# supernomad/quantum

Hardware: AMD Instinct MI355X
Metric: AES-256-GCM seal+unseal GiB/s (device-resident packets) at 1/2/4/8 MI355X (higher is better)
Workload: dtype u8

## Files before the change

quantum_amd/csrc/gcm_kernels.hip:

```cpp
#include <hip/hip_runtime.h>
#include <stdint.h>

#include <algorithm>

#include "gcm_internal.h"

namespace qgcm {

typedef __attribute__((address_space(3))) uint32_t lds_u32;
typedef uint32_t u32x4 __attribute__((ext_vector_type(4)));
typedef __attribute__((address_space(3))) u32x4 lds_u128;

struct __attribute__((aligned(4))) W4 {
    uint32_t x, y, z, w;
};

#ifndef QGCM_NT_DATA
#define QGCM_NT_DATA 0
#endif
typedef uint32_t u32x4u __attribute__((ext_vector_type(4), aligned(4)));
__device__ __forceinline__ W4 load_block(const W4 *p) {
    if constexpr ((QGCM_NT_DATA & 1) != 0) {
        const u32x4u v = __builtin_nontemporal_load(reinterpret_cast<const u32x4u *>(p));
        return W4{v.x, v.y, v.z, v.w};
// ... 257 lines not shown
        }
        *(lds_u64 *)(size_t)(512u * i + 8u * v) = u32x2{a0, a1};
        *(lds_u64 *)(size_t)(512u * i + 256u + 8u * v) = u32x2{a2, a3};
    }
}

struct Tab2F {
    Keys kk;
    TT<kG5Bytes, true> t;
    uint32_t mf8;
    __device__ __forceinline__ void setup(Ctr &c, uint32_t n0, uint32_t n1, uint32_t n2, uint32_t hi) const {
        ctr_setup(c, n0, n1, n2, hi, kk, t);
    }
    __device__ __forceinline__ void block(const Ctr &c, uint32_t lo, uint32_t &k0, uint32_t &k1, uint32_t &k2,
                                          uint32_t &k3) const {
        ctr_block_t<TT<kG5Bytes, true>, kG5Bytes>(c, lo, kk, t, k0, k1, k2, k3);
    }
    __device__ __forceinline__ void ghash(uint32_t &y0, uint32_t &y1, uint32_t &y2, uint32_t &y3, uint32_t) const {
        ghash_mul5(y0, y1, y2, y3, mf8);
    }
};

__device__ __forceinline__ uint32_t vreg(uint32_t x) {
    asm volatile("" : "+v"(x));
    return x;
}

template <bool kFence = true>
__device__ __forceinline__ void ghash_mul(uint32_t &y0, uint32_t &y1, uint32_t &y2, uint32_t &y3, uint32_t gb) {
    uint32_t a0 = 0, a1 = 0, a2 = 0, a3 = 0;
    const uint32_t yw[4] = {y0, y1, y2, y3};
#pragma unroll
    for (int w = 0; w < 4; ++w) {
        const uint32_t hi = yw[w] & 0xf0f0f0f0u;
        const uint32_t lo = (yw[w] << 4) & 0xf0f0f0f0u;
#pragma unroll
        for (int k = 0; k < 4; ++k) {
            const int j = 4 * w + k;
            const uint4 th = lds128(perm(gb, hi, 0x0c060500u | k) + (2 * j) * 256);
            const uint4 tl = lds128(perm(gb, lo, 0x0c060500u | k) + (2 * j + 1) * 256);
            a0 = xor3(a0, th.x, tl.x);
            a1 = xor3(a1, th.y, tl.y);
            a2 = xor3(a2, th.z, tl.z);
            a3 = xor3(a3, th.w, tl.w);
        }
        if constexpr (kFence) asm volatile("" : "+v"(a0), "+v"(a1), "+v"(a2), "+v"(a3)::"memory");
    }
    y0 = a0;
    y1 = a1;
    y2 = a2;
    y3 = a3;
}

__device__ __forceinline__ void ghash_mul_global(uint32_t &y0, uint32_t &y1, uint32_t &y2, uint32_t &y3,
                                                 const uint4 *__restrict__ T) {
    uint32_t a0 = 0, a1 = 0, a2 = 0, a3 = 0;
    const uint32_t yw[4] = {y0, y1, y2, y3};
    const char *base = reinterpret_cast<const char *>(T);
#pragma unroll
    for (int w = 0; w < 4; ++w) {
#pragma unroll
        for (int k = 0; k < 4; ++k) {
            const int j = 4 * w + k;
            const uint32_t oh = (yw[w] >> (8 * k)) & 0xf0u;
            const uint32_t ol = ((yw[w] >> (8 * k)) & 0x0fu) << 4;
            const uint4 th = *reinterpret_cast<const uint4 *>(base + (2 * j) * 256 + oh);
            const uint4 tl = *reinterpret_cast<const uint4 *>(base + (2 * j + 1) * 256 + ol);
            a0 = xor3(a0, th.x, tl.x);
            a1 = xor3(a1, th.y, tl.y);
            a2 = xor3(a2, th.z, tl.z);
            a3 = xor3(a3, th.w, tl.w);
        }
        asm volatile("" : "+v"(a0), "+v"(a1), "+v"(a2), "+v"(a3)::"memory");
    }
    y0 = a0;
    y1 = a1;
    y2 = a2;
    y3 = a3;
}

__device__ __forceinline__ void ghash_lenblock_global(uint32_t aad_len, uint32_t L, const uint4 *__restrict__ T,
                                                      uint32_t &y0, uint32_t &y1, uint32_t &y2, uint32_t &y3) {
    const char *base = reinterpret_cast<const char *>(T);
    const uint32_t w1 = bswap(aad_len * 8u), w3 = bswap(L * 8u);
    const uint32_t v[5] = {w1 >> 24, w3, w3 >> 8, w3 >> 16, w3 >> 24};
    const int j[5] = {7, 12, 13, 14, 15};
    uint32_t a0 = 0, a1 = 0, a2 = 0, a3 = 0;
#pragma unroll
    for (int i = 0; i < 5; ++i) {
        const uint4 th = *reinterpret_cast<const uint4 *>(base + (2 * j[i]) * 256 + (v[i] & 0xf0u));
        const uint4 tl = *reinterpret_cast<const uint4 *>(base + (2 * j[i] + 1) * 256 + ((v[i] & 0x0fu) << 4));
        a0 = xor3(a0, th.x, tl.x);
        a1 = xor3(a1, th.y, tl.y);
        a2 = xor3(a2, th.z, tl.z);
        a3 = xor3(a3, th.w, tl.w);
    }
    y0 = a0;
    y1 = a1;
    y2 = a2;
    y3 = a3;
}

__device__ __forceinline__ uint32_t sel4(uint32_t q, uint32_t a, uint32_t b, uint32_t c, uint32_t d) {
    return q == 0 ? a : (q == 1 ? b : (q == 2 ? c : d));
}
__device__ __forceinline__ uint32_t lowmask(uint32_t s) { return s ? (0xffffffffu >> (32 - 8 * s)) : 0u; }
__device__ __forceinline__ void store_bytes(uint8_t *p, uint32_t v, uint32_t nbytes) {
    if (nbytes > 0) p[0] = (uint8_t)v;
    if (nbytes > 1) p[1] = (uint8_t)(v >> 8);
    if (nbytes > 2) p[2] = (uint8_t)(v >> 16);
}
__device__ __forceinline__ uint32_t load_bytes(const uint8_t *p, uint32_t nbytes) {
    uint32_t v = 0;
    if (nbytes > 0) v |= p[0];
    if (nbytes > 1) v |= (uint32_t)p[1] << 8;
    if (nbytes > 2) v |= (uint32_t)p[2] << 16;
    return v;
}


__device__ __forceinline__ void read_tail(const uint8_t *data, uint32_t L, uint32_t &g0, uint32_t &g1, uint32_t &g2,
                                          uint32_t &g3, uint32_t &n0, uint32_t &n1, uint32_t &n2) {
    const uint32_t s = L & 3u;
    const uint32_t *t = reinterpret_cast<const uint32_t *>(data + (L & ~3u));
    const uint32_t w0 = t[0], w1 = t[1], w2 = t[2], w3 = t[3], w4 = t[4], w5 = t[5], w6 = t[6];
    const uint32_t w7 = load_bytes(data + (L & ~3u) + 28, s);
    g0 = __builtin_amdgcn_alignbyte(w1, w0, s);
    g1 = __builtin_amdgcn_alignbyte(w2, w1, s);
    g2 = __builtin_amdgcn_alignbyte(w3, w2, s);
    g3 = __builtin_amdgcn_alignbyte(w4, w3, s);
    n0 = __builtin_amdgcn_alignbyte(w5, w4, s);
    n1 = __builtin_amdgcn_alignbyte(w6, w5, s);
    n2 = __builtin_amdgcn_alignbyte(w7, w6, s);
}

__device__ __forceinline__ void read_nonce(const uint8_t *data, uint32_t L, uint32_t &n0, uint32_t &n1, uint32_t &n2) {
    const uint32_t s = L & 3u;
    const uint32_t *t = reinterpret_cast<const uint32_t *>(data + (L & ~3u));
    const uint32_t w4 = t[4], w5 = t[5], w6 = t[6];
    const uint32_t w7 = load_bytes(data + (L & ~3u) + 28, s);
    n0 = __builtin_amdgcn_alignbyte(w5, w4, s);
    n1 = __builtin_amdgcn_alignbyte(w6, w5, s);
    n2 = __builtin_amdgcn_alignbyte(w7, w6, s);
}
// ... 77 lines not shown
        const W4 &c = kSeal ? out : in;
        eng.ghash(z0, z1, z2, z3, gH4);
        z0 ^= c.x;
        z1 ^= c.y;
        z2 ^= c.z;
        z3 ^= c.w;
        blast = (int)bi;
    }
    const bool part = r && (nfull & 3u) == m;
    if (part || m == (d & 3u)) {
        const uint32_t ctr = part ? nfull + 2 : 1u;
        if ((ctr >> 8) != hi) {
            hi = ctr >> 8;
            eng.setup(cc, n0, n1, n2, hi);
        }
        uint32_t k0, k1, k2, k3;
        eng.block(cc, ctr & 0xffu, k0, k1, k2, k3);
        if (part) {
            uint8_t *blk = data + 16u * nfull;
            const W4 in = *reinterpret_cast<const W4 *>(blk);
            const uint32_t q = r >> 2, sb = r & 3u;
            const uint32_t o0 = in.x ^ k0, o1 = in.y ^ k1, o2 = in.z ^ k2, o3 = in.w ^ k3;
            uint32_t *bw = reinterpret_cast<uint32_t *>(blk);
            if (q > 0) bw[0] = o0;
            if (q > 1) bw[1] = o1;
            if (q > 2) bw[2] = o2;
            const uint32_t oq = sel4(q, o0, o1, o2, o3) & lowmask(sb);
            W4 c = kSeal ? W4{o0, o1, o2, o3} : in;
            if (kSeal)
                prefix = oq;
            else
                store_bytes(blk + 4 * q, oq, sb);
            c.x &= q > 0 ? 0xffffffffu : lowmask(sb);
            c.y &= q > 1 ? 0xffffffffu : (q == 1 ? lowmask(sb) : 0u);
            c.z &= q > 2 ? 0xffffffffu : (q == 2 ? lowmask(sb) : 0u);
            c.w &= q == 3 ? lowmask(sb) : 0u;
            eng.ghash(z0, z1, z2, z3, gH4);
            z0 ^= c.x;
            z1 ^= c.y;
            z2 ^= c.z;
            z3 ^= c.w;
            blast = (int)nfull;
        } else {
            e0 = k0;
            e1 = k1;
            e2 = k2;
            e3 = k3;
        }
    }
    }
    {
        const uint32_t em = d + 1u - (uint32_t)blast;
        const uint32_t tsel = em == 2 ? kGhH2 : em == 3 ? kGhH3 : em == 4 ? kGhH4 : kGhH5;
        ghash_mul_global(z0, z1, z2, z3, Hg + tsel);
        uint32_t l0, l1, l2, l3;
        ghash_lenblock_global(b.aad_len, L, Hg, l0, l1, l2, l3);
        z0 = quad_xor(z0) ^ l0;
        z1 = quad_xor(z1) ^ l1;
        z2 = quad_xor(z2) ^ l2;
        z3 = quad_xor(z3) ^ l3;
    }
    e0 = quad_xor(e0);
    e1 = quad_xor(e1);
    e2 = quad_xor(e2);
    e3 = quad_xor(e3);
    const uint32_t t0 = z0 ^ e0, t1 = z1 ^ e1, t2 = z2 ^ e2, t3 = z3 ^ e3;
    const uint32_t owner = r ? (nfull & 3u) : 0u;
    if (kSeal) {
        if (m == owner) {
            write_tail(data, L, t0, t1, t2, t3, n0, n1, n2, prefix);
            if (b.status) b.status[pkt] = 1;
        }
    } else {
        read_tag(data, L, g0, g1, g2, g3);
        const bool ok = ((t0 ^ g0) | (t1 ^ g1) | (t2 ^ g2) | (t3 ^ g3)) == 0;
        if (!ok) {
            for (uint32_t bi = m; bi < nfull; bi += 4) {
                const W4 zz = {0, 0, 0, 0};
                *reinterpret_cast<W4 *>(data + 16u * bi) = zz;
            }
            if (r && m == owner) {
                uint32_t *bw = reinterpret_cast<uint32_t *>(data + 16u * nfull);
                for (uint32_t w = 0; w < (r >> 2); ++w) bw[w] = 0;
                store_bytes(data + 16u * nfull + (r & ~3u), 0, r & 3u);
            }
        }
        if (b.status && m == 0) b.status[pkt] = ok ? 1 : 0;
    }
}

#ifndef QGCM_TILE_POOL
#define QGCM_TILE_POOL 4
#endif
#ifndef QGCM_TAIL_EIGHTHS
#define QGCM_TAIL_EIGHTHS 4
#endif
constexpr uint32_t kPoolCtr = kG5Bytes + kTeBytes;

#ifdef QGCM_QUAD_STATS
__device__ unsigned long long g_quad_stats[4096 * 8];
#endif

template <bool kDesc>
constexpr int quad_waves() { return kDesc ? 12 : 16; }
template <bool kDesc>
constexpr int quad_wpe() { return kDesc ? 3 : 8; }

template <bool kSeal, bool kDesc>
__global__ void __launch_bounds__(quad_waves<kDesc>() * 64) __attribute__((amdgpu_waves_per_eu(quad_wpe<kDesc>(),
                                                                                                  quad_wpe<kDesc>())))
gcm_quad_kernel(Batch b, const uint32_t *__restrict__ rk_table) {
    constexpr uint32_t kW = quad_waves<kDesc>();
    constexpr uint32_t kT = kW * 64;
    constexpr uint32_t kTeBase = kDesc ? 0u : kG5Bytes;
    const uint32_t lane = threadIdx.x & 63u;
    const uint32_t wave = threadIdx.x >> 6;
    const uint32_t m = lane & 3u;
    const uint32_t qd = lane >> 2;
    if (kDesc && b.tile_list && __builtin_amdgcn_readfirstlane(*b.n_list) == 0) return;

    for (uint32_t i = threadIdx.x; i < kTeBytes / 4; i += kT) {
        const uint32_t x = i >> 6, slot = i & 63u;
        lds_st32(kTeBase + 4 * i, b.te[(slot >> 5) * 256u + x]);
    }
    if constexpr (!kDesc) g5_fill(b.gh_table + (size_t)b.uniform_key * kGhEntries + kGhH4, threadIdx.x, kT);
    if constexpr (!kDesc && QGCM_TILE_POOL) {
        if (threadIdx.x == 0) lds_st32(kPoolCtr, kW);
    }
#if QGCM_TILE_POOL == 4
    if constexpr (!kDesc) {
        if (threadIdx.x == 0) lds_st32(kPoolCtr + 12, 0u);
    }
#endif
    __syncthreads();

    const uint32_t lb = (lane & 31u) << 2;
    const uint32_t m8 = vreg(0x0000ff00u), mf8 = vreg(0x000000f8u);
    const uint32_t gH4 = kDesc ? kTeBytes + wave * kGhBytes : 0u;
    uint32_t cur_key = kDesc ? 0xffffffffu : b.uniform_key;
    const uint32_t ntiles = kDesc ? (b.tile_list ? *b.n_list : b.n_items >> 4) : ((b.n + 15) >> 4);

#ifdef QGCM_QUAD_STATS
    unsigned long long *qs = g_quad_stats + (size_t)blockIdx.x * 8u;
    uint32_t qs_tiles = 0;
    if (!kDesc && threadIdx.x == 0) {
        qs[0] = wall_clock64();
        qs[4] = __builtin_amdgcn_s_getreg((31 << 11) | 20);
        qs[5] = __builtin_amdgcn_s_getreg((31 << 11) | 4);
    }
#endif
#ifdef QGCM_QUAD_STATS
#define QS_TILE() ++qs_tiles
#define QS_END()                                                  \
    do {                                                          \
        if (!kDesc && lane == 0) {                                \
            const unsigned long long t_ = wall_clock64();         \
            atomicMax(&qs[1], t_);                                \
            atomicAdd(&qs[2], t_);                                \
            atomicAdd(&qs[3], (unsigned long long)qs_tiles);      \
            atomicMax(&qs[6], (1ull << 62) - t_);                 \
        }                                                         \
    } while (0)
#else
#define QS_TILE() do { } while (0)
#define QS_END() do { } while (0)
#endif
#if QGCM_TILE_POOL == 4
    uint32_t sidx = 0xffffffffu, tail0 = 0;
    if constexpr (!kDesc) {
        const uint32_t rows = ntiles / (gridDim.x * kW);
        if (b.pool && rows > 0) {
            const uint32_t tail_rows = rows < 2 ? 0u : std::min(rows - 1u, std::max(1u, rows * QGCM_TAIL_EIGHTHS / 8u));
            sidx = (rows - tail_rows) * kW;
            tail0 = (rows - tail_rows) * gridDim.x * kW;
        }
    }
#endif
    uint32_t tile = blockIdx.x * kW + wave;
    if constexpr (kDesc) {
        uint32_t t = 0;
        if (lane == 0) t = atomicAdd(b.tile_counter, 1u);
        tile = __builtin_amdgcn_readfirstlane(__shfl(t, 0));
    }
    for (; tile < ntiles;) {
        uint32_t pkt, L;
        bool valid;
        uint64_t off;
        uint32_t wkey = cur_key;
        if constexpr (kDesc) {
            const uint32_t wt = b.tile_list ? b.tile_list[tile] : tile;
            pkt = b.worklist[wt * 16u + qd];
            valid = pkt != 0xffffffffu;
            qgcm_desc dsc = {0, 0, 0};
            if (valid) dsc = b.descs[pkt];
            off = dsc.offset;
            L = kSeal ? dsc.len : dsc.len - QGCM_OVERHEAD;
            const uint64_t vmask = __ballot(valid);
            if (vmask != 0) {
                wkey = __builtin_amdgcn_readfirstlane(__shfl(dsc.key_idx, __ffsll((unsigned long long)vmask) - 1));
                if (wkey != cur_key) {
                    const uint4 *src = b.gh_table + (size_t)wkey * kGhEntries + kGhH4;
#pragma unroll
                    for (int r = 0; r < 8; ++r) {
                        const uint32_t e = r * 64 + lane;
                        lds_st_comb(gH4, e, src[e]);
                    }
                    __builtin_amdgcn_fence(__ATOMIC_RELEASE, "wavefront");
                    __builtin_amdgcn_wave_barrier();
                    __builtin_amdgcn_fence(__ATOMIC_ACQUIRE, "wavefront");
                    cur_key = wkey;
                }
            }
            uint32_t t = 0;
            if (lane == 0) t = atomicAdd(b.tile_counter, 1u);
            const uint32_t next = __builtin_amdgcn_readfirstlane(__shfl(t, 0));
            asm volatile("" : "+v"(L));
            if (!valid) {
                tile = next;
                continue;
            }
            tile = next;
        } else {
            pkt = tile * 16u + qd;
            L = b.uniform_len;
            asm volatile("" : "+s"(L));
            valid = pkt < b.n;
            if (!kSeal) {
                if (L < (uint32_t)QGCM_OVERHEAD) valid = false;
                L -= QGCM_OVERHEAD;
            }
            off = (uint64_t)pkt * b.stride;
            if constexpr (QGCM_TILE_POOL) {
                uint32_t i = 0;
                if (lane == 0) i = __atomic_fetch_add((lds_u32 *)(size_t)kPoolCtr, 1u, __ATOMIC_RELAXED);
                i = __builtin_amdgcn_readfirstlane(i);
                tile = blockIdx.x * kW + (i % kW) + (i / kW) * gridDim.x * kW;
#if QGCM_TILE_POOL == 4
                if (i >= sidx) {
                    uint32_t c = 0;
                    if (lane == 0) c = atomicAdd(b.pool, 1u);
                    tile = tail0 + __builtin_amdgcn_readfirstlane(c);
                }
#endif
            } else {
                tile += gridDim.x * kW;
            }
            if (!valid) {
                if (!kSeal && b.status && pkt < b.n && m == 0) b.status[pkt] = 0;
                continue;
            }
        }
        const Keys kk = {rk_table + (size_t)wkey * kRkWords, rk_table + (size_t)wkey * kRkWords + 64};
        if constexpr (kDesc) {
            quad_packet<kSeal>(b, Tab2{kk, {lb, m8}}, pkt, off, L, wkey, m, gH4);
        } else {
            quad_packet<kSeal>(b, Tab2F{kk, {lb, m8}, mf8}, pkt, off, L, wkey, m, gH4);
        }
        QS_TILE();
    }
    QS_END();
#if QGCM_TILE_POOL == 4
    if constexpr (!kDesc) {
        if (b.pool) {
            uint32_t last = 0;
            if (lane == 0 && __atomic_fetch_add((lds_u32 *)(size_t)(kPoolCtr + 12), 1u, __ATOMIC_RELAXED) == kW - 1) {
                __threadfence();
                last = atomicAdd(b.pool + kPoolDoneWord, 1u) == gridDim.x - 1u ? 1u : 0u;
            }
            if (lane == 0 && last) {
                __threadfence();
                b.pool[0] = 0;
                b.pool[kPoolDoneWord] = 0;
                __threadfence_system();
                __hip_atomic_store(b.pool_done, b.pool_gen, __ATOMIC_RELEASE, __HIP_MEMORY_SCOPE_SYSTEM);
            }
        }
    }
#endif
}
#undef QS_TILE
#undef QS_END

#ifdef QGCM_QUAD_STATS
extern "C" int qgcm_debug_quad_stats(unsigned long long *out, int n, int reset) {
    if (n > 4096 * 8) n = 4096 * 8;
    if (hipMemcpyFromSymbol(out, HIP_SYMBOL(g_quad_stats), (size_t)n * 8) != hipSuccess) return -1;
    if (reset) {
        static unsigned long long zero[4096 * 8];
        if (hipMemcpyToSymbol(HIP_SYMBOL(g_quad_stats), zero, sizeof(zero)) != hipSuccess) return -1;
    }
    return 0;
}
#endif

constexpr uint32_t kSegCtl = kG5Bytes + kTeBytes;
constexpr uint32_t kSegLds = kSegCtl + 16u;
constexpr uint32_t kSegDone = 0xffffffffu;

__device__ __forceinline__ volatile lds_u32 *seg_ctl(uint32_t i) { return (volatile lds_u32 *)(size_t)(kSegCtl + 4u * i); }

template <class P>
__device__ __forceinline__ uint32_t wave_lower_bound(uint32_t lo, uint32_t hi, uint32_t lane, P pred) {
    while (hi - lo > 63u) {
        const uint32_t step = (hi - lo + 62u) / 63u;
        const uint32_t p = min(lo + lane * step, hi);
        const uint64_t msk = __ballot(pred(p));
        const uint32_t f = (uint32_t)__ffsll((unsigned long long)msk) - 1u;
        if (f == 0) return lo;
        const uint32_t nlo = lo + (f - 1u) * step + 1u, nhi = min(lo + f * step, hi);
        lo = nlo;
        hi = nhi;
    }
    const uint64_t msk = __ballot(pred(min(lo + lane, hi)));
    return lo + (uint32_t)__ffsll((unsigned long long)msk) - 1u;
}

#ifdef QGCM_SEG_STATS
__device__ unsigned long long g_seg_stats[4096 * 16];
#define SEG_STAT_ADD(i, v) \
    do { if (lane == 0) atomicAdd(&g_seg_stats[blockIdx.x * 16u + (i)], (unsigned long long)(v)); } while (0)
#define SEG_NOW() wall_clock64()
#else
#define SEG_STAT_ADD(i, v) do { } while (0)
#define SEG_NOW() 0ull
#endif

#ifndef QGCM_SEG_START
#define QGCM_SEG_START 1
#endif
#ifndef QGCM_SEG_HELP_MIN
#define QGCM_SEG_HELP_MIN 16
#endif
#ifndef QGCM_SEG_LAST
// ... 1270 lines not shown
```

quantum_amd/csrc/qgcm_api.cpp:

```cpp
#include <hip/hip_runtime.h>
#include <errno.h>
#include <stdint.h>
#include <stdio.h>
#include <stdlib.h>
#include <string.h>
#include <sys/random.h>

#include <algorithm>
#include <atomic>
#include <chrono>
#include <memory>
#include <future>
#include <map>
#include <mutex>
#include <thread>
#include <vector>

#include "../../include/qgcm.h"
#include "chain_claim.h"
#include "gcm_internal.h"

using namespace qgcm;

constexpr int kPipeStreams = 3;
constexpr uint64_t kPipeChunk = 32ull << 20;
constexpr uint64_t kHostChunk = 64ull << 20;
constexpr uint64_t kHostRing = 4ull << 30;

struct qgcm_ctx {
    int device = 0;
    int num_cus = 0;
    uint32_t max_keys = 0;
    int uniform_variant = kVariantUniform;
    int desc_variant = kVariantDescQuad;
    int wgs_per_cu_override = 0;
    bool one_kernel = true;
    bool variant_forced = false;
    uint32_t desc_one_max = kDescOneMax;
    uint32_t direct_max = kDirectMax;
    uint32_t one_uniform_max = kOneUniformMax;
    uint32_t launch_chunk = kLaunchChunk;
    uint32_t desc_chunk = kDescChunk;
    bool desc_one_on = true, host_direct = true, small_wl = true;
    uint64_t chain_chunk = kPipeChunk;
    int chain_slots = kPipeStreams, chain_dev_ahead = 2, chain_dev_backlog = -1;
    bool snappy_group = true;
    int snappy_per_cu = 0;
    bool chain_pin = true;
    std::mutex codec_cpus_mu;
    std::vector<int> codec_cpus;
    uint32_t *d_rk = nullptr;
    uint4 *d_gh = nullptr;
    uint4 *d_pw = nullptr;
    uint32_t pw_keys = 0;
    uint32_t *d_te = nullptr;
    uint8_t *d_sbox = nullptr;
    uint8_t *d_key_valid = nullptr;
    std::vector<uint8_t> key_set;
    std::mutex key_mu;

    std::mutex ws_mu;
    void *d_qws = nullptr;
    size_t qws_cap = 0;

    std::mutex io_mu;
    struct OneSlot {
        std::mutex mu;
        hipStream_t stream = nullptr;
        uint8_t *h = nullptr;
        size_t cap = 0;
    };
    static constexpr int kOneSlots = 8;
    static constexpr size_t kOneSlotCap = kOneCap + 4096;
    static_assert((kOneCap - 16u) + 16u <= kOneSlotCap, "record, tail and status bytes fit a pooled staging slot");
    static_assert(one_fits_launch(16336, true, QGCM_MAX_AAD) && !one_fits_launch(16337, true, QGCM_MAX_AAD) &&
                      one_record_bytes(16336, true) + one_tail_bytes(QGCM_MAX_AAD) + 16u <= kOneSlotCap,
                  "the largest long-AAD call fits a pooled staging slot");
    OneSlot one[kOneSlots];
    OneSlot big;
    std::atomic<uint32_t> one_rr{0};

    hipStream_t pipe[kPipeStreams] = {};
    std::vector<hipEvent_t> ev_in, ev_kern, ev_out;
    uint64_t host_chunk = kHostChunk, host_ring = kHostRing;
    uint8_t *d_ring = nullptr;
    size_t ring_cap = 0;
    uint8_t *h_stat = nullptr;
    size_t hstat_cap = 0;
// ... 32 lines not shown

int env_int(const char *name, int dflt) {
    const char *v = getenv(name);
    return v && *v ? atoi(v) : dflt;
}

uint8_t gf8_mul(uint8_t a, uint8_t b) {
    uint8_t p = 0;
    for (int i = 0; i < 8; ++i) {
        if (b & 1) p ^= a;
        const uint8_t hi = a & 0x80;
        a <<= 1;
        if (hi) a ^= 0x1b;
        b >>= 1;
    }
    return p;
}

void build_tables(uint8_t sbox[256], uint32_t te[512]) {
    for (int x = 0; x < 256; ++x) {
        uint8_t inv = 0;
        if (x) {
            uint8_t r = 1, b = (uint8_t)x;
            for (int e = 254; e; e >>= 1) {
                if (e & 1) r = gf8_mul(r, b);
                b = gf8_mul(b, b);
            }
            inv = r;
        }
        auto rl = [](uint8_t v, int s) { return (uint8_t)((v << s) | (v >> (8 - s))); };
        sbox[x] = inv ^ rl(inv, 1) ^ rl(inv, 2) ^ rl(inv, 3) ^ rl(inv, 4) ^ 0x63;
    }
    for (int x = 0; x < 256; ++x) {
        const uint32_t s = sbox[x], s2 = gf8_mul((uint8_t)s, 2), s3 = s2 ^ s;
        const uint32_t t0 = s2 | (s << 8) | (s << 16) | (s3 << 24);
        te[x] = t0;
        te[256 + x] = (t0 << 8) | (t0 >> 24);
    }
}

void set_err(char *err, int errlen, const char *msg) {
    if (err && errlen > 0) snprintf(err, (size_t)errlen, "%s", msg);
}

int hip_fail(hipError_t e) { return e == hipSuccess ? QGCM_OK : QGCM_E_HIP; }

int grid_for(const qgcm_ctx *ctx, uint32_t n_items, int variant) {
    const int cus = std::max(1, ctx->num_cus - resident_workers_running(ctx->res.load(std::memory_order_acquire)));
    const uint32_t waves = (uint32_t)variant_waves(variant);
    const uint32_t tiles = (n_items + 15) / 16;
    const uint32_t wgs = (tiles + waves - 1) / waves;
    const uint32_t per_cu = ctx->wgs_per_cu_override > 0 ? (uint32_t)ctx->wgs_per_cu_override
                                                         : (uint32_t)variant_wgs_per_cu(variant);
    const uint32_t cap = (uint32_t)cus * per_cu;
    return (int)(wgs < cap ? (wgs ? wgs : 1) : cap);
}

Batch base_batch(const qgcm_ctx *ctx) {
    Batch b{};
    b.rk_table = ctx->d_rk;
    b.gh_table = ctx->d_gh;
    b.pw_table = ctx->d_pw;
    b.pw_keys = ctx->pw_keys;
    b.te = ctx->d_te;
    b.key_valid = ctx->d_key_valid;
    b.max_keys = ctx->max_keys;
    return b;
}

int run_uniform(qgcm_ctx *ctx, bool seal, uint8_t *arena, uint64_t stride, uint32_t n, uint32_t len,
                uint32_t key_idx, const uint8_t *nonces, uint32_t aad_len, uint8_t *status, hipStream_t s);

int run_one(qgcm_ctx *ctx, bool seal, uint8_t *slot, uint64_t stride, uint32_t len, uint32_t key_idx,
            uint32_t aad_len, uint8_t *status, hipStream_t s) {
    if (ctx->one_kernel && stride + one_tail_bytes(aad_len) <= kOneCap - 16 && !(stride & 15) &&
        !((uintptr_t)slot & 15)) {
        volatile uint8_t *done = status + 1;
        *done = 0;
        Batch b = base_batch(ctx);
        b.done = status + 1;
        b.arena = slot;
        b.status = status;
        b.stride = stride;
        b.uniform_len = len;
        b.uniform_key = key_idx;
        b.n = 1;
        b.n_items = 64;
        b.aad_len = aad_len;
        if (launch_one(seal, b, s) != hipSuccess) return QGCM_E_HIP;
        ctx->count(QGCM_KERNEL_ONE);
        const auto t0 = std::chrono::steady_clock::now();
        for (uint32_t spins = 0; *done == 0; ++spins) {
            __builtin_ia32_pause();
            if ((spins & 1023) == 1023 && std::chrono::steady_clock::now() - t0 > std::chrono::seconds(1)) break;
        }
        if (*done == 0) return hip_fail(hipStreamSynchronize(s));
        std::atomic_thread_fence(std::memory_order_acquire);
        return QGCM_OK;
    }
    if (aad_len > 4) return QGCM_E_ARG;
    const int rc = run_uniform(ctx, seal, slot, stride, 1, len, key_idx, nullptr, aad_len, status, s);
    return rc == QGCM_OK ? hip_fail(hipStreamSynchronize(s)) : rc;
}

Resident *get_resident(qgcm_ctx *ctx) {
    Resident *r = ctx->res.load(std::memory_order_acquire);
    if (r || !ctx->res_on || ctx->res_failed.load(std::memory_order_relaxed)) return r;
// ... 311 lines not shown
        case QGCM_E_AUTH: return "message authentication failed";
        case QGCM_E_NOMEM: return "out of device or pinned memory";
        default: return "unknown error";
    }
}

qgcm_ctx *qgcm_create(int device, uint32_t max_keys, char *err, int errlen) {
    (void)tl_dummy;
    if (max_keys == 0 || max_keys > QGCM_MAX_KEYS) {
        set_err(err, errlen, "max_keys must be in [1, 2^20 - 1]");
        return nullptr;
    }
    int ndev = 0;
    if (hipGetDeviceCount(&ndev) != hipSuccess || device < 0 || device >= ndev) {
        set_err(err, errlen, "no such HIP device");
        return nullptr;
    }
    if (hipSetDevice(device) != hipSuccess) {
        set_err(err, errlen, "hipSetDevice failed");
        return nullptr;
    }
    hipDeviceProp_t prop;
    if (hipGetDeviceProperties(&prop, device) != hipSuccess) {
        set_err(err, errlen, "hipGetDeviceProperties failed");
        return nullptr;
    }
    if (strncmp(prop.gcnArchName, "gfx950", 6) != 0) {
        char m[QGCM_ERRLEN];
        snprintf(m, sizeof m, "device %d is %s; libqgcm is built for gfx950 only", device, prop.gcnArchName);
        set_err(err, errlen, m);
        return nullptr;
    }
    {
        static std::mutex init_mu;
        std::lock_guard<std::mutex> g(init_mu);
        if (init_kernels() != hipSuccess) {
            set_err(err, errlen, "kernel setup failed");
            return nullptr;
        }
    }
    auto *ctx = new qgcm_ctx();
    ctx->device = device;
    ctx->num_cus = prop.multiProcessorCount;
    ctx->max_keys = max_keys;
    ctx->key_set.assign(max_keys, 0);
    if (const char *v = getenv("QGCM_VARIANT")) {
        const int iv = atoi(v);
        if (variant_valid(iv) && !variant_desc(iv)) {
            ctx->uniform_variant = iv;
            ctx->variant_forced = true;
        }
    }
    if (const char *v = getenv("QGCM_WGS_PER_CU")) ctx->wgs_per_cu_override = atoi(v);
    if (const char *v = getenv("QGCM_ONE_KERNEL")) ctx->one_kernel = atoi(v) != 0;
    if (const char *v = getenv("QGCM_CHAIN_DEVICE")) ctx->chain_codec = std::max(0, std::min(2, atoi(v)));
    if (const char *v = getenv("QGCM_RESIDENT")) ctx->res_on = atoi(v) != 0;
    ctx->res_cfg = qgcm::resident_config_from_env();
    if (const char *v = getenv("QGCM_ONE_UNIFORM_MAX")) ctx->one_uniform_max = (uint32_t)std::max(0, atoi(v));
    if (const char *v = getenv("QGCM_DESC_ONE_MAX")) ctx->desc_one_max = (uint32_t)std::max(0, atoi(v));
    if (const char *v = getenv("QGCM_DIRECT_MAX")) ctx->direct_max = (uint32_t)std::max(0, atoi(v));
    if (const char *v = getenv("QGCM_LAUNCH_CHUNK"))
        ctx->launch_chunk = (uint32_t)std::max(0, atoi(v)) & ~63u;
    if (const char *v = getenv("QGCM_DESC_CHUNK")) ctx->desc_chunk = (uint32_t)std::max(0, atoi(v));
    if (const char *v = getenv("QGCM_PIPE_CHUNK_MB")) ctx->host_chunk = (uint64_t)std::max(1, atoi(v)) << 20;
    if (const char *v = getenv("QGCM_PIPE_RING_MB")) ctx->host_ring = (uint64_t)std::max(1, atoi(v)) << 20;
    if (const char *v = getenv("QGCM_DESC_VARIANT")) {
        const int iv = atoi(v);
        if (variant_valid(iv) && variant_desc(iv)) ctx->desc_variant = iv;
    }
    auto off = [](const char *name) {
        const char *v = getenv(name);
        return v && !strcmp(v, "0");
    };
    ctx->chain_chunk = (uint64_t)std::max(1, env_int("QGCM_CHAIN_CHUNK_MB", (int)(kPipeChunk >> 20))) << 20;
    ctx->chain_slots = std::max(1, std::min(16, env_int("QGCM_CHAIN_SLOTS", kPipeStreams)));
    ctx->chain_dev_ahead = std::max(1, env_int("QGCM_CHAIN_DEV_AHEAD", 2));
    ctx->chain_dev_backlog = env_int("QGCM_CHAIN_DEV_BACKLOG", -1);
    ctx->snappy_group = env_int("QGCM_SNAPPY_GROUP", 1) != 0;
    ctx->snappy_per_cu = std::max(0, env_int("QGCM_SNAPPY_PER_CU", 0));
    ctx->chain_pin = env_int("QGCM_CHAIN_PIN", 1) != 0;
    ctx->desc_one_on = !off("QGCM_DESC_ONE");
    ctx->host_direct = !off("QGCM_HOST_DIRECT");
    ctx->small_wl = !off("QGCM_SMALL_WORKLIST");
    uint8_t sbox[256];
    uint32_t te[512];
    build_tables(sbox, te);
    bool ok = hipMalloc(&ctx->d_rk, (size_t)max_keys * kRkWords * 4) == hipSuccess &&
              hipMalloc(&ctx->d_gh, (size_t)max_keys * kGhEntries * 16) == hipSuccess &&
              hipMalloc(&ctx->d_key_valid, max_keys) == hipSuccess &&
              hipMemset(ctx->d_rk, 0, (size_t)max_keys * kRkWords * 4) == hipSuccess &&
              hipMemset(ctx->d_gh, 0, (size_t)max_keys * kGhEntries * 16) == hipSuccess &&
              hipMemset(ctx->d_key_valid, 0, max_keys) == hipSuccess &&
              hipMalloc(&ctx->d_te, sizeof te) == hipSuccess && hipMalloc(&ctx->d_sbox, sizeof sbox) == hipSuccess &&
              hipMemcpy(ctx->d_te, te, sizeof te, hipMemcpyHostToDevice) == hipSuccess &&
              hipMemcpy(ctx->d_sbox, sbox, sizeof sbox, hipMemcpyHostToDevice) == hipSuccess &&
              hipEventCreateWithFlags(&ctx->ws_done, hipEventDisableTiming) == hipSuccess;
    ctx->pw_keys = (uint32_t)std::min<int64_t>(max_keys, std::max(0, env_int("QGCM_FLAT_GHASH_KEYS", 256)));
    if (ok && ctx->pw_keys &&
        (hipMalloc(&ctx->d_pw, (size_t)ctx->pw_keys * kPwPowers * kPwEntries * 16) != hipSuccess ||
         hipMemset(ctx->d_pw, 0, (size_t)ctx->pw_keys * kPwPowers * kPwEntries * 16) != hipSuccess)) {
        hipFree(ctx->d_pw);
        ctx->d_pw = nullptr;
        ctx->pw_keys = 0;
    }
    for (int k = 0; ok && k < kPipeStreams; ++k)
        ok = hipStreamCreateWithFlags(&ctx->pipe[k], hipStreamNonBlocking) == hipSuccess;
// ... 792 lines not shown
```

Baseline: 876.2.

## Specialise uniform GCM tile loop with hoisted length block and optional paired tails

Splits the uniform-length path out of the shared quad kernel loop into a dedicated uniform_tiles routine. The GHASH length block, identical for every packet, is now computed once per wave and kept in scalar registers instead of being recomputed per packet. The new routine also adds an optional mode (off by default) that starts the next tile's packet on idle lanes during a one-block tail, handing state over with DPP permutes. A grid-size cap environment knob is added, and GHASH table addressing is changed to a base pointer plus byte offset.

```diff
diff --git a/quantum_amd/csrc/gcm_kernels.hip b/quantum_amd/csrc/gcm_kernels.hip
--- a/quantum_amd/csrc/gcm_kernels.hip
+++ b/quantum_amd/csrc/gcm_kernels.hip
@@ -333,11 +333,13 @@
     y3 = a3;
 }
 
+__device__ __forceinline__ uint4 gh_row(const uint4 *__restrict__ G, uint32_t off) {
+    return *reinterpret_cast<const uint4 *>(reinterpret_cast<const char *>(G) + off);
+}
 __device__ __forceinline__ void ghash_mul_global(uint32_t &y0, uint32_t &y1, uint32_t &y2, uint32_t &y3,
-                                                 const uint4 *__restrict__ T) {
+                                                 const uint4 *__restrict__ G, uint32_t toff) {
     uint32_t a0 = 0, a1 = 0, a2 = 0, a3 = 0;
     const uint32_t yw[4] = {y0, y1, y2, y3};
-    const char *base = reinterpret_cast<const char *>(T);
 #pragma unroll
     for (int w = 0; w < 4; ++w) {
 #pragma unroll
@@ -345,8 +347,8 @@
             const int j = 4 * w + k;
             const uint32_t oh = (yw[w] >> (8 * k)) & 0xf0u;
             const uint32_t ol = ((yw[w] >> (8 * k)) & 0x0fu) << 4;
-            const uint4 th = *reinterpret_cast<const uint4 *>(base + (2 * j) * 256 + oh);
-            const uint4 tl = *reinterpret_cast<const uint4 *>(base + (2 * j + 1) * 256 + ol);
+            const uint4 th = gh_row(G, toff + oh + (2 * j) * 256);
+            const uint4 tl = gh_row(G, toff + ol + (2 * j + 1) * 256);
             a0 = xor3(a0, th.x, tl.x);
             a1 = xor3(a1, th.y, tl.y);
             a2 = xor3(a2, th.z, tl.z);
@@ -360,17 +362,16 @@
     y3 = a3;
 }
 
-__device__ __forceinline__ void ghash_lenblock_global(uint32_t aad_len, uint32_t L, const uint4 *__restrict__ T,
+__device__ __forceinline__ void ghash_lenblock_global(uint32_t aad_len, uint32_t L, const uint4 *__restrict__ G,
                                                       uint32_t &y0, uint32_t &y1, uint32_t &y2, uint32_t &y3) {
-    const char *base = reinterpret_cast<const char *>(T);
     const uint32_t w1 = bswap(aad_len * 8u), w3 = bswap(L * 8u);
     const uint32_t v[5] = {w1 >> 24, w3, w3 >> 8, w3 >> 16, w3 >> 24};
     const int j[5] = {7, 12, 13, 14, 15};
     uint32_t a0 = 0, a1 = 0, a2 = 0, a3 = 0;
 #pragma unroll
     for (int i = 0; i < 5; ++i) {
-        const uint4 th = *reinterpret_cast<const uint4 *>(base + (2 * j[i]) * 256 + (v[i] & 0xf0u));
-        const uint4 tl = *reinterpret_cast<const uint4 *>(base + (2 * j[i] + 1) * 256 + ((v[i] & 0x0fu) << 4));
+        const uint4 th = gh_row(G, kGhH * 16u + (2 * j[i]) * 256 + (v[i] & 0xf0u));
+        const uint4 tl = gh_row(G, kGhH * 16u + (2 * j[i] + 1) * 256 + ((v[i] & 0x0fu) << 4));
         a0 = xor3(a0, th.x, tl.x);
         a1 = xor3(a1, th.y, tl.y);
         a2 = xor3(a2, th.z, tl.z);
@@ -554,7 +555,7 @@
     {
         const uint32_t em = d + 1u - (uint32_t)blast;
         const uint32_t tsel = em == 2 ? kGhH2 : em == 3 ? kGhH3 : em == 4 ? kGhH4 : kGhH5;
-        ghash_mul_global(z0, z1, z2, z3, Hg + tsel);
+        ghash_mul_global(z0, z1, z2, z3, Hg, tsel * 16u);
         uint32_t l0, l1, l2, l3;
         ghash_lenblock_global(b.aad_len, L, Hg, l0, l1, l2, l3);
         z0 = quad_xor(z0) ^ l0;
@@ -607,6 +608,263 @@
 constexpr int quad_waves() { return kDesc ? 12 : 16; }
 template <bool kDesc>
 constexpr int quad_wpe() { return kDesc ? 3 : 8; }
+
+#ifndef QGCM_PAIR_TAIL
+#define QGCM_PAIR_TAIL 0
+#endif
+
+template <uint32_t kW>
+__device__ __forceinline__ uint32_t uniform_next_tile(const Batch &b, uint32_t tile, uint32_t lane, uint32_t sidx,
+                                                      uint32_t tail0) {
+    if constexpr (QGCM_TILE_POOL) {
+        uint32_t i = 0;
+        if (lane == 0) i = __atomic_fetch_add((lds_u32 *)(size_t)kPoolCtr, 1u, __ATOMIC_RELAXED);
+        i = __builtin_amdgcn_readfirstlane(i);
+        uint32_t t = blockIdx.x * kW + (i % kW) + (i / kW) * gridDim.x * kW;
+#if QGCM_TILE_POOL == 4
+        if (i >= sidx) {
+            uint32_t c = 0;
+            if (lane == 0) c = atomicAdd(b.pool, 1u);
+            t = tail0 + __builtin_amdgcn_readfirstlane(c);
+        }
+#endif
+        return t;
+    } else {
+        return tile + gridDim.x * kW;
+    }
+}
+
+template <int kPerm>
+__device__ __forceinline__ uint32_t quad_perm(uint32_t v) {
+    return (uint32_t)__builtin_amdgcn_mov_dpp((int)v, kPerm, 0xf, 0xf, false);
+}
+
+template <bool kSeal, uint32_t kW>
+__device__ __forceinline__ uint32_t uniform_tiles(const Batch &b, const Tab2F &eng, uint32_t lane, uint32_t wave,
+                                                  uint32_t ntiles, uint32_t sidx, uint32_t tail0) {
+    const uint32_t m = lane & 3u, qd = lane >> 2;
+    const uint4 *G = b.gh_table + (size_t)b.uniform_key * kGhEntries;
+    uint32_t done = 0;
+    uint32_t lh0, lh1, lh2, lh3;
+    {
+        const uint32_t Lp = kSeal ? b.uniform_len : b.uniform_len - (uint32_t)QGCM_OVERHEAD;
+        ghash_lenblock_global(b.aad_len, Lp, G, lh0, lh1, lh2, lh3);
+        lh0 = __builtin_amdgcn_readfirstlane(lh0);
+        lh1 = __builtin_amdgcn_readfirstlane(lh1);
+        lh2 = __builtin_amdgcn_readfirstlane(lh2);
+        lh3 = __builtin_amdgcn_readfirstlane(lh3);
+    }
+    uint64_t off = 0;
+    uint32_t n0 = 0, n1 = 0, n2 = 0, hi = 0;
+    uint32_t z0 = 0, z1 = 0, z2 = 0, z3 = 0;
+    uint32_t e0 = 0, e1 = 0, e2 = 0, e3 = 0;
+    int blast = -1;
+    Ctr cc = {0, 0, 0, 0, 0, 0};
+    bool rot = false;
+    for (uint32_t tile = blockIdx.x * kW + wave; tile < ntiles;) {
+        uint32_t L = b.uniform_len;
+        asm volatile("" : "+s"(L));
+        const uint32_t next = uniform_next_tile<kW>(b, tile, lane, sidx, tail0);
+        const uint32_t pkt = tile * 16u + qd;
+        bool valid = pkt < b.n;
+        if (!kSeal) {
+            if (L < (uint32_t)QGCM_OVERHEAD) valid = false;
+            L -= QGCM_OVERHEAD;
+        }
+        if (!valid) {
+            if (!kSeal && b.status && pkt < b.n && m == 0) b.status[pkt] = 0;
+            tile = next;
+            continue;
+        }
+        const uint32_t nfull = L >> 4, r = L & 15u;
+        const uint32_t d = nfull + (r ? 1u : 0u);
+        const uint32_t s = rot ? 2u : 0u;
+        uint32_t prefix = 0;
+        e0 = e1 = e2 = e3 = 0;
+        if (!rot) {
+            off = (uint64_t)pkt * b.stride + 4;
+            if (kSeal && b.nonces) {
+                const uint32_t *np = reinterpret_cast<const uint32_t *>(b.nonces + 12ull * pkt);
+                n0 = np[0];
+                n1 = np[1];
+                n2 = np[2];
+            } else {
+                read_nonce(b.arena + off, L, n0, n1, n2);
+            }
+            z0 = z1 = z2 = z3 = 0;
+            if (m == 3 && b.aad_len)
+                z0 = *reinterpret_cast<const uint32_t *>(b.arena + off - 4) & (b.aad_len >= 4 ? 0xffffffffu : lowmask(b.aad_len));
+            blast = -1;
+            hi = 0;
+            eng.setup(cc, n0, n1, n2, 0);
+        }
+        uint32_t bi = s + m;
+        const uint32_t nfast = (nfull - s) >> 2;
+        for (uint32_t p = 0; p < nfast; ++p, bi += 4) {
+            const uint32_t ctr = bi + 2;
+            if ((ctr >> 8) != hi) {
+                hi = ctr >> 8;
+                eng.setup(cc, n0, n1, n2, hi);
+            }
+            W4 *p4 = reinterpret_cast<W4 *>(b.arena + off + 16u * bi);
+            const W4 in = load_block(p4);
+            uint32_t k0, k1, k2, k3;
+            eng.block(cc, ctr & 0xffu, k0, k1, k2, k3);
+            const W4 out = {in.x ^ k0, in.y ^ k1, in.z ^ k2, in.w ^ k3};
+            store_block(p4, out);
+            const W4 &c = kSeal ? out : in;
+            eng.ghash(z0, z1, z2, z3, 0);
+            z0 ^= c.x;
+            z1 ^= c.y;
+            z2 ^= c.z;
+            z3 ^= c.w;
+        }
+        if (nfast) blast = (int)bi - 4;
+        const uint32_t base = s + 4u * nfast;
+        const bool pair = QGCM_PAIR_TAIL && !rot && d - base == 1u && nfull >= 2u && next < ntiles &&
+                          next * 16u + 16u <= b.n && tile * 16u + 16u <= b.n;
+        const bool ahead = pair && m >= 2u;
+        if (ahead) {
+            const uint32_t pn = next * 16u + qd;
+            off = (uint64_t)pn * b.stride + 4;
+            if (kSeal && b.nonces) {
+                const uint32_t *np = reinterpret_cast<const uint32_t *>(b.nonces + 12ull * pn);
+                n0 = np[0];
+                n1 = np[1];
+                n2 = np[2];
+            } else {
+                read_nonce(b.arena + off, L, n0, n1, n2);
+            }
+            hi = 0;
+            eng.setup(cc, n0, n1, n2, 0);
+            bi = m - 2u;
+        }
+        for (uint32_t gb = base; gb <= d; gb += 4, bi += 4) {
+            if (bi > d) continue;
+            const bool j0 = !ahead && bi == d, part = !ahead && r && bi == nfull;
+            const uint32_t ctr = j0 ? 1u : bi + 2;
+            if ((ctr >> 8) != hi) {
+                hi = ctr >> 8;
+                eng.setup(cc, n0, n1, n2, hi);
+            }
+            W4 *p4 = reinterpret_cast<W4 *>(b.arena + off + 16u * bi);
+            W4 in = {0, 0, 0, 0};
+            if (!j0) in = *p4;
+            uint32_t k0, k1, k2, k3;
+            eng.block(cc, ctr & 0xffu, k0, k1, k2, k3);
+            const uint32_t o0 = in.x ^ k0, o1 = in.y ^ k1, o2 = in.z ^ k2, o3 = in.w ^ k3;
+            W4 c = kSeal ? W4{o0, o1, o2, o3} : in;
+            if (j0) {
+                e0 = k0;
+                e1 = k1;
+                e2 = k2;
+                e3 = k3;
+            } else if (part) {
+                const uint32_t q = r >> 2, sb = r & 3u;
+                uint32_t *bw = reinterpret_cast<uint32_t *>(p4);
+                if (q > 0) bw[0] = o0;
+                if (q > 1) bw[1] = o1;
+                if (q > 2) bw[2] = o2;
+                const uint32_t oq = sel4(q, o0, o1, o2, o3) & lowmask(sb);
+                if (kSeal)
+                    prefix = oq;
+                else
+                    store_bytes(reinterpret_cast<uint8_t *>(p4) + 4 * q, oq, sb);
+                c.x &= q > 0 ? 0xffffffffu : lowmask(sb);
+                c.y &= q > 1 ? 0xffffffffu : (q == 1 ? lowmask(sb) : 0u);
+                c.z &= q > 2 ? 0xffffffffu : (q == 2 ? lowmask(sb) : 0u);
+                c.w &= q == 3 ? lowmask(sb) : 0u;
+            } else {
+                *p4 = W4{o0, o1, o2, o3};
+            }
+            if (ahead) {
+                e0 = c.x;
+                e1 = c.y;
+                e2 = c.z;
+                e3 = c.w;
+            } else if (!j0) {
+                eng.ghash(z0, z1, z2, z3, 0);
+                z0 ^= c.x;
+                z1 ^= c.y;
+                z2 ^= c.z;
+                z3 ^= c.w;
+                blast = (int)bi;
+            }
+        }
+        {
+            const uint32_t em = d + 1u - (uint32_t)blast;
+            const uint32_t tsel = em == 2 ? kGhH2 : em == 3 ? kGhH3 : em == 4 ? kGhH4 : kGhH5;
+            ghash_mul_global(z0, z1, z2, z3, G, tsel * 16u);
+            z0 = quad_xor(z0) ^ lh0;
+            z1 = quad_xor(z1) ^ lh1;
+            z2 = quad_xor(z2) ^ lh2;
+            z3 = quad_xor(z3) ^ lh3;
+        }
+        uint32_t t0, t1, t2, t3;
+        if (pair) {
+            t0 = z0 ^ quad_perm<0x55>(e0);
+            t1 = z1 ^ quad_perm<0x55>(e1);
+            t2 = z2 ^ quad_perm<0x55>(e2);
+            t3 = z3 ^ quad_perm<0x55>(e3);
+        } else {
+            t0 = z0 ^ quad_xor(e0);
+            t1 = z1 ^ quad_xor(e1);
+            t2 = z2 ^ quad_xor(e2);
+            t3 = z3 ^ quad_xor(e3);
+        }
+        const uint32_t owner = ((r ? nfull : 0u) - s) & 3u;
+        if (kSeal) {
+            if (m == owner) {
+                write_tail(b.arena + off, L, t0, t1, t2, t3, n0, n1, n2, prefix);
+                if (b.status) b.status[pkt] = 1;
+            }
+        } else {
+            uint32_t g0, g1, g2, g3;
+            read_tag(b.arena + off, L, g0, g1, g2, g3);
+            uint32_t bad = (t0 ^ g0) | (t1 ^ g1) | (t2 ^ g2) | (t3 ^ g3);
+            bad = quad_perm<0x00>(bad);
+            if (bad) {
+                uint32_t mz = m, zero = 0;
+                asm volatile("" : "+v"(mz), "+v"(zero));
+                uint8_t *dz = b.arena + (uint64_t)(tile * 16u + (lane >> 2)) * b.stride + 4;
+                const W4 zz = {zero, zero, zero, zero};
+                for (uint32_t bj = s + mz; bj < nfull; bj += 4) *reinterpret_cast<W4 *>(dz + 16u * bj) = zz;
+                if (s && mz >= 2u) *reinterpret_cast<W4 *>(dz + 16u * (mz - 2u)) = zz;
+                if (r && mz == owner) {
+                    uint32_t *bw = reinterpret_cast<uint32_t *>(dz + 16u * nfull);
+                    for (uint32_t w = 0; w < (r >> 2); ++w) bw[w] = zero;
+                    store_bytes(dz + 16u * nfull + (r & ~3u), zero, r & 3u);
+                }
+            }
+            if (b.status && m == 0) b.status[pkt] = bad ? 0 : 1;
+        }
+        ++done;
+        if (pair) {
+            off = ((uint64_t)quad_perm<0xEE>((uint32_t)(off >> 32)) << 32) | quad_perm<0xEE>((uint32_t)off);
+            n0 = quad_perm<0xEE>(n0);
+            n1 = quad_perm<0xEE>(n1);
+            n2 = quad_perm<0xEE>(n2);
+            cc.K0 = quad_perm<0xEE>(cc.K0);
+            cc.U0 = quad_perm<0xEE>(cc.U0);
+            cc.U1 = quad_perm<0xEE>(cc.U1);
+            cc.U2 = quad_perm<0xEE>(cc.U2);
+            cc.U3 = quad_perm<0xEE>(cc.U3);
+            hi = 0;
+            z0 = m >= 2u ? e0 : 0u;
+            z1 = m >= 2u ? e1 : 0u;
+            z2 = m >= 2u ? e2 : 0u;
+            z3 = m >= 2u ? e3 : 0u;
+            if (m == 1 && b.aad_len)
+                z0 = *reinterpret_cast<const uint32_t *>(b.arena + off - 4) & (b.aad_len >= 4 ? 0xffffffffu : lowmask(b.aad_len));
+            uint32_t mo = m;
+            asm volatile("" : "+v"(mo));
+            blast = mo >= 2u ? (int)mo - 2 : -1;
+        }
+        rot = pair;
+        tile = next;
+    }
+    return done;
+}
 
 template <bool kSeal, bool kDesc>
 __global__ void __launch_bounds__(quad_waves<kDesc>() * 64) __attribute__((amdgpu_waves_per_eu(quad_wpe<kDesc>(),
@@ -652,7 +910,6 @@
     }
 #endif
 #ifdef QGCM_QUAD_STATS
-#define QS_TILE() ++qs_tiles
 #define QS_END()                                                  \
     do {                                                          \
         if (!kDesc && lane == 0) {                                \
@@ -664,11 +921,10 @@
         }                                                         \
     } while (0)
 #else
-#define QS_TILE() do { } while (0)
 #define QS_END() do { } while (0)
 #endif
+    uint32_t sidx = 0xffffffffu, tail0 = 0;
 #if QGCM_TILE_POOL == 4
-    uint32_t sidx = 0xffffffffu, tail0 = 0;
     if constexpr (!kDesc) {
         const uint32_t rows = ntiles / (gridDim.x * kW);
         if (b.pool && rows > 0) {
@@ -678,25 +934,26 @@
         }
     }
 #endif
-    uint32_t tile = blockIdx.x * kW + wave;
-    if constexpr (kDesc) {
-        uint32_t t = 0;
-        if (lane == 0) t = atomicAdd(b.tile_counter, 1u);
-        tile = __builtin_amdgcn_readfirstlane(__shfl(t, 0));
-    }
-    for (; tile < ntiles;) {
-        uint32_t pkt, L;
-        bool valid;
-        uint64_t off;
-        uint32_t wkey = cur_key;
-        if constexpr (kDesc) {
+    if constexpr (!kDesc) {
+        const Keys kk = {rk_table + (size_t)cur_key * kRkWords, rk_table + (size_t)cur_key * kRkWords + 64};
+        [[maybe_unused]] const uint32_t ndone =
+            uniform_tiles<kSeal, kW>(b, Tab2F{kk, {lb, m8}, mf8}, lane, wave, ntiles, sidx, tail0);
+#ifdef QGCM_QUAD_STATS
+        qs_tiles = ndone;
+#endif
+    } else {
+        uint32_t tile = 0;
+        if (lane == 0) tile = atomicAdd(b.tile_counter, 1u);
+        tile = __builtin_amdgcn_readfirstlane(__shfl(tile, 0));
+        for (; tile < ntiles;) {
+            uint32_t wkey = cur_key;
             const uint32_t wt = b.tile_list ? b.tile_list[tile] : tile;
-            pkt = b.worklist[wt * 16u + qd];
-            valid = pkt != 0xffffffffu;
+            const uint32_t pkt = b.worklist[wt * 16u + qd];
+            const bool valid = pkt != 0xffffffffu;
             qgcm_desc dsc = {0, 0, 0};
             if (valid) dsc = b.descs[pkt];
-            off = dsc.offset;
-            L = kSeal ? dsc.len : dsc.len - QGCM_OVERHEAD;
+            const uint64_t off = dsc.offset;
+            uint32_t L = kSeal ? dsc.len : dsc.len - QGCM_OVERHEAD;
             const uint64_t vmask = __ballot(valid);
             if (vmask != 0) {
                 wkey = __builtin_amdgcn_readfirstlane(__shfl(dsc.key_idx, __ffsll((unsigned long long)vmask) - 1));
@@ -717,59 +974,23 @@
             if (lane == 0) t = atomicAdd(b.tile_counter, 1u);
             const uint32_t next = __builtin_amdgcn_readfirstlane(__shfl(t, 0));
             asm volatile("" : "+v"(L));
-            if (!valid) {
-                tile = next;
-                continue;
-            }
             tile = next;
-        } else {
-            pkt = tile * 16u + qd;
-            L = b.uniform_len;
-            asm volatile("" : "+s"(L));
-            valid = pkt < b.n;
-            if (!kSeal) {
-                if (L < (uint32_t)QGCM_OVERHEAD) valid = false;
-                L -= QGCM_OVERHEAD;
-            }
-            off = (uint64_t)pkt * b.stride;
-            if constexpr (QGCM_TILE_POOL) {
-                uint32_t i = 0;
-                if (lane == 0) i = __atomic_fetch_add((lds_u32 *)(size_t)kPoolCtr, 1u, __ATOMIC_RELAXED);
-                i = __builtin_amdgcn_readfirstlane(i);
-                tile = blockIdx.x * kW + (i % kW) + (i / kW) * gridDim.x * kW;
-#if QGCM_TILE_POOL == 4
-                if (i >= sidx) {
-                    uint32_t c = 0;
-                    if (lane == 0) c = atomicAdd(b.pool, 1u);
-                    tile = tail0 + __builtin_amdgcn_readfirstlane(c);
-                }
-#endif
-            } else {
-                tile += gridDim.x * kW;
-            }
-            if (!valid) {
-                if (!kSeal && b.status && pkt < b.n && m == 0) b.status[pkt] = 0;
-                continue;
-            }
-        }
-        const Keys kk = {rk_table + (size_t)wkey * kRkWords, rk_table + (size_t)wkey * kRkWords + 64};
-        if constexpr (kDesc) {
+            if (!valid) continue;
+            const Keys kk = {rk_table + (size_t)wkey * kRkWords, rk_table + (size_t)wkey * kRkWords + 64};
             quad_packet<kSeal>(b, Tab2{kk, {lb, m8}}, pkt, off, L, wkey, m, gH4);
-        } else {
-            quad_packet<kSeal>(b, Tab2F{kk, {lb, m8}, mf8}, pkt, off, L, wkey, m, gH4);
-        }
-        QS_TILE();
+        }
     }
     QS_END();
 #if QGCM_TILE_POOL == 4
     if constexpr (!kDesc) {
         if (b.pool) {
             uint32_t last = 0;
-            if (lane == 0 && __atomic_fetch_add((lds_u32 *)(size_t)(kPoolCtr + 12), 1u, __ATOMIC_RELAXED) == kW - 1) {
+            const bool lane0 = __builtin_amdgcn_mbcnt_hi(~0u, __builtin_amdgcn_mbcnt_lo(~0u, 0u)) == 0;
+            if (lane0 && __atomic_fetch_add((lds_u32 *)(size_t)(kPoolCtr + 12), 1u, __ATOMIC_RELAXED) == kW - 1) {
                 __threadfence();
                 last = atomicAdd(b.pool + kPoolDoneWord, 1u) == gridDim.x - 1u ? 1u : 0u;
             }
-            if (lane == 0 && last) {
+            if (lane0 && last) {
                 __threadfence();
                 b.pool[0] = 0;
                 b.pool[kPoolDoneWord] = 0;
@@ -780,7 +1001,6 @@
     }
 #endif
 }
-#undef QS_TILE
 #undef QS_END
 
 #ifdef QGCM_QUAD_STATS
diff --git a/quantum_amd/csrc/qgcm_api.cpp b/quantum_amd/csrc/qgcm_api.cpp
--- a/quantum_amd/csrc/qgcm_api.cpp
+++ b/quantum_amd/csrc/qgcm_api.cpp
@@ -34,6 +34,7 @@
     int uniform_variant = kVariantUniform;
     int desc_variant = kVariantDescQuad;
     int wgs_per_cu_override = 0;
+    int grid_wgs = 0;
     bool one_kernel = true;
     bool variant_forced = false;
     uint32_t desc_one_max = kDescOneMax;
@@ -172,7 +173,8 @@
     const uint32_t wgs = (tiles + waves - 1) / waves;
     const uint32_t per_cu = ctx->wgs_per_cu_override > 0 ? (uint32_t)ctx->wgs_per_cu_override
                                                          : (uint32_t)variant_wgs_per_cu(variant);
-    const uint32_t cap = (uint32_t)cus * per_cu;
+    uint32_t cap = (uint32_t)cus * per_cu;
+    if (ctx->grid_wgs > 0) cap = std::min(cap, (uint32_t)ctx->grid_wgs);
     return (int)(wgs < cap ? (wgs ? wgs : 1) : cap);
 }
 
@@ -590,6 +592,7 @@
         }
     }
     if (const char *v = getenv("QGCM_WGS_PER_CU")) ctx->wgs_per_cu_override = atoi(v);
+    if (const char *v = getenv("QGCM_GRID_WGS")) ctx->grid_wgs = std::max(0, atoi(v));
     if (const char *v = getenv("QGCM_ONE_KERNEL")) ctx->one_kernel = atoi(v) != 0;
     if (const char *v = getenv("QGCM_CHAIN_DEVICE")) ctx->chain_codec = std::max(0, std::min(2, atoi(v)));
     if (const char *v = getenv("QGCM_RESIDENT")) ctx->res_on = atoi(v) != 0;
```

Measured after the change: 877.1 (median of 2 runs). No clear change (+0.1%).
